# Plachtaa/FAcodec

Hardware: AMD Instinct MI355X
Metric: 24kHz audio sec encoded+decoded per wall-sec (higher is better)
Workload: dtype f32; 1 GPU; configs[1]: batch=32/GPU x 2 s @ 24 kHz, forward encoder->FVQ(6 codebooks)->decoder, FAcodec configs/config.yml model (137.7 M params), weights formula-generated, weight-norm re-materialised every step; clips_per_gpu=32, samples_per_clip=48000, parallelism=dp1 (independent clips, no collective)

## Files before the change

facodec_amd/_lib.py:

```python
import ctypes as C
import os

_HERE = os.path.dirname(os.path.abspath(__file__))
LIB_PATH = os.environ.get("FAC_LIB_PATH", os.path.join(_HERE, "libfacodec_hip.so"))

PAD_ZERO, PAD_REFLECT = 0, 1
ACT_NONE, ACT_TANH, ACT_MISH, ACT_LOG_MEL = 0, 1, 2, 3
ACT_GATE, ACT_WN_RES_SKIP = 4, 5

_p = C.c_void_p
_i = C.c_int
_i64 = C.c_int64
_f = C.c_float


class ConvDesc(C.Structure):
    _fields_ = [
        ("x", _p), ("w", _p), ("bias", _p), ("alpha_in", _p), ("alpha_out", _p), ("res", _p), ("y", _p), ("y2", _p), ("alpha_y2", _p), ("w_k1", _p), ("bias_k1", _p),
        ("x_bs", _i64), ("x_cs", _i64), ("y_bs", _i64), ("y_cs", _i64),
        ("B", C.c_int32), ("C_in", C.c_int32), ("T_in", C.c_int32), ("C_out", C.c_int32),
        ("C_out_pad", C.c_int32), ("T_out", C.c_int32),
        ("K", C.c_int32), ("stride", C.c_int32), ("dilation", C.c_int32), ("pad_left", C.c_int32),
        ("pad_mode", C.c_int32), ("n_phase", C.c_int32), ("y_tstride", C.c_int32), ("phase_shift", C.c_int32),
        ("act", C.c_int32),
        ("w_batched", C.c_int32), ("w_bs", _i64), ("ws", _p), ("ws_bytes", _i64), ("w_split", _p),
        ("K1", C.c_int32), ("dilation2", C.c_int32), ("row_phases", C.c_int32),
        ("x_p8", _p), ("x_p8_plane_bytes", _i64), ("y2_p8", _p), ("y2_p8_plane_bytes", _i64),
        ("pw_split", C.c_int32), ("split_rows", C.c_int32),
        ("gate_cond", _p), ("gate_cond_bs", _i64),
        ("keep_tile160", C.c_int32),
    ]


class VqDesc(C.Structure):
    _fields_ = [
        ("residual", _p), ("z_in", _p), ("zq_acc", _p), ("zq_out", _p), ("w_in", _p), ("b_in", _p),
        ("codebook", _p), ("w_out", _p), ("w_out_scale", _p), ("b_out", _p), ("mask", _p), ("codes", _p), ("z_e", _p),
        ("loss_part", _p), ("codes_bs", _i64),
        ("B", C.c_int32), ("D", C.c_int32), ("T", C.c_int32), ("Kc", C.c_int32),
    ]



VQ_DECODE_MAX_Q = 16


class VqDecodeDesc(C.Structure):
    _fields_ = [
        ("codes", _p * 3), ("codes_bs", _i64 * 3), ("codes_qs", _i64 * 3), ("n_q", C.c_int32 * 3),
        ("codebook", _p * VQ_DECODE_MAX_Q), ("w_out", _p * VQ_DECODE_MAX_Q), ("w_out_scale", _p * VQ_DECODE_MAX_Q),
        ("b_out", _p * VQ_DECODE_MAX_Q), ("style", _p), ("outs", _p), ("z", _p * 3),
        ("B", C.c_int32), ("D", C.c_int32), ("T", C.c_int32), ("Kc", C.c_int32),
    ]
# ... 120 lines not shown
    "fac_snake_bwd": (_i, [_p, _p, _p, _p, _p, _p, _i, _i, _i, _p]),
    "fac_pack_lstm_whh_t": (_i, [_p, _p, _i, _p]),
    "fac_lstm_layer_bwd": (_i, [_p, _p, _p, _p, _p, _p, _i, _i, _i, _p]),
    "fac_to_p8": (_i, [_p, _p, _p, _i, _i, _i, _p]),
    "fac_lstm_persist_ok": (_i, [_i, _i]),
    "fac_lstm_persist_stream_ok": (_i, [_p]),
    "fac_pack_lstm_whh16": (_i, [_p, _p, _i, _i, _p]),
    "fac_lstm_layer_fwd_persist": (_i, [_p, _p, _p, _p, _p, _p, _i, _i, _i, _i, _p]),
    "fac_lstm_layer_bwd_persist": (_i, [_p, _p, _p, _p, _p, _p, _i, _i, _i, _i, _p]),
    "fac_lstm_persist_split_ok": (_i, [_i, _i]),
    "fac_lstm_persist_timeouts": (_i, []),
    "fac_lstm_persist_arm": (_i, [_p]),
    "fac_lstm_abort_flag": (_i, [_p, _p]),
    "fac_mask_flags_if": (_i, [_p, _i, _p, _p]),
    "fac_pack_lstm_whh_split": (_i, [_p, _p, _i, _p]),
    "fac_lstm_layer_fwd_persist_split": (_i, [_p, _p, _p, _p, _i, _i, _i, _i, _p]),
    "fac_snake_bwd_fused": (_i, [_p, _p, _p, _p, _p, _p, _p, _p, _i, _i, _i, _p]),
    "fac_bias_grad": (_i, [_p, _p, _p, _i, _i, _i, _p]),
    "fac_snake_bwd_fused_rs": (_i, [_p, _p, _p, _i64, _p, _p, _p, _p, _p, _i, _i, _i, _p]),
    "fac_pad_fold_edges": (_i, [_p, _i, _i, _i, _i, _i, _p]),
    "fac_pack_convtr_w": (_i, [_p, _p, _p, _i, _i, _i, _i, _p]),
    "fac_conv1d_fwd": (_i, [C.POINTER(ConvDesc), _p]),
    "fac_conv1d_variant": (_i, [C.POINTER(ConvDesc), C.c_char_p, _i]),
    "fac_snake_fwd": (_i, [_p, _p, _p, _i, _i, _i, _p]),
    "fac_lstm_to_time_major": (_i, [_p, _p, _i, _i, _i, _p]),
    "fac_lstm_from_time_major": (_i, [_p, _p, _p, _p, _i, _i, _i, _p]),
    "fac_pack_lstm_whh": (_i, [_p, _p, _i, _p]),
    "fac_lstm_layer_fwd": (_i, [_p, _p, _p, _p, _i, _i, _i, _p]),
    "fac_lstm_layer_fwd_from": (_i, [_p, _p, _p, _p, _i, _i, _i, _i64, _p]),
    "fac_lstm_layer_fwd_train": (_i, [_p, _p, _p, _p, _p, _p, _i, _i, _i, _i64, _p]),
    "fac_lstm_gate_bwd": (_i, [_p, _p, _p, _p, _p, _p, _p, _i, _i, _i64, _i, _p]),
    "fac_tanh_bwd": (_i, [_p, _p, _p, _i64, _p]),
    "fac_pair_bwd": (_i, [_p, _p, _p, _i64, _i, C.c_float, C.c_float, _i, _p]),
    "fac_spec_power_bwd": (_i, [_p, _p, _p, _i, _i, _i, _i, _p]),
    "fac_stft_frames_bwd": (_i, [_p, _p, _i, _i, _i, _i, _i, _i, _i, _p]),
    "fac_vq_latent_bwd": (_i, [_p, _p, _p, _i64, _p, _p, _p, _p, _i, _i, _p]),
    "fac_vq_codebook_grad": (_i, [_p, _p, _p, _i64, _p, _p, _i, _i, _i, _i, _p]),
    "fac_layernorm_c_affine_bwd": (_i, [_p, _p, _p, _p, _p, _p, _i, _i, _i, _p]),
    "fac_rows_fma": (_i, [_p, _p, _p, _p, _i, _i64, _f, _p]),
    "fac_grad_norm_clip": (_i, [_p, _i64, _f, _p, _p, _p]),
    "fac_adamw_step": (_i, [_p, _p, _p, _p, _i64, _f, _f, _f, _f, _f, _i64, _p, _p]),
    "fac_logdiff_rms_bwd": (_i, [_p, _p, _p, _i, _i, _i, _f, _f, _i, _p]),
    "fac_gather_copy": (_i, [_p, _p, _p, _i, _p]),
    "fac_adamw_step_masked": (_i, [_p, _p, _p, _p, _i64, _p, _i, _p, _p, _p, _f, _f, _f, _f, _f, _p, _p]),
    "fac_gate_bwd": (_i, [_p, _p, _p, _i, _i, _i, _p]),
    "fac_mish_fwd": (_i, [_p, _p, _i64, _p]),
# ... 119 lines not shown
```

facodec_amd/build.py:

```python
import os
import subprocess
import sys
from concurrent.futures import ThreadPoolExecutor

HERE = os.path.dirname(os.path.abspath(__file__))
CSRC = os.path.join(HERE, "csrc")
TAG = os.environ.get("FAC_BUILD_TAG", "")
LIB = os.path.join(HERE, "libfacodec_hip%s.so" % ("_" + TAG if TAG else ""))
OBJDIR = "build" + ("_" + TAG if TAG else "")
SOURCES = ["conv1d_api.hip", "conv1d_tile_128x128.hip", "conv1d_tile_96x128.hip", "conv1d_tile_64x128.hip",
           "conv1d_tile_32x256.hip", "conv1d_tile_128x32.hip", "conv1d_tile_128x256.hip", "conv1d_fused_ru.hip", "conv1d_narrow.hip", "conv1d_pw.hip", "conv1d_pw_split.hip", "conv1d_skinny.hip", "conv1d_bsplit.hip", "conv1d_bsplit96.hip", "conv1d_gemm_split.hip", "conv1d_bsplit2.hip", "conv1d_bwd.hip", "conv1d_wgrad_split.hip", "conv1d_wgrad_k1.hip", "train_misc.hip", "optim.hip", "train_quant.hip", "train_pred.hip", "train_disc.hip", "train_redecoder.hip", "pack.hip", "prep_batch.hip", "lstm.hip", "lstm_persist.hip", "vq.hip", "vq_decode.hip", "bitpack.hip", "misc.hip", "attention_stream.hip", "attention_tiled.hip","ragged.hip", "resample.hip", "loudness.hip", "metrics.hip", "stream_pool.hip", "plc.hip", "jdc.hip", "rccl_arena.hip"]
FLAGS = ["--offload-arch=gfx950", "-O3", "-std=c++17", "-fPIC", "-ffp-contract=off",
         "-Wno-unused-result"] + os.environ.get("FAC_EXTRA_FLAGS", "").split()


def _hipcc():
    for cand in (os.environ.get("HIPCC"), "/opt/rocm/bin/hipcc", "hipcc"):
        if cand and (os.path.isabs(cand) and os.path.exists(cand) or not os.path.isabs(cand)):
            return cand
    return "hipcc"


def _stale(target, deps):
    if not os.path.exists(target):
        return True
    tt = os.path.getmtime(target)
    return any(os.path.getmtime(d) > tt for d in deps)


def build_lib(force=False, verbose=True):
    hipcc = _hipcc()
    headers = sorted(os.path.join(CSRC, f) for f in os.listdir(CSRC) if f.endswith(".h")) + [os.path.join(HERE, "..", "include", "facodec_hip.h")]
    objs, jobs = [], []
    os.makedirs(os.path.join(CSRC, OBJDIR), exist_ok=True)
# ... 23 lines not shown
```

facodec_amd/csrc/conv1d_api.hip:

```cpp
#include "conv1d_mfma.h"
#include <stdlib.h>

namespace fac {

enum ConvKernel : int {
  CK_128x32 = 0,
  CK_32x256 = 1,
  CK_64x128 = 2,
  CK_96x128 = 3,
  CK_128x128 = 4,
  CK_128x256 = 5,
  CK_96x256 = 6,
  CK_FUSED_RU = 7,
  CK_128x160 = 8,
  CK_NARROW = 9,
  CK_SKINNY = 10,
  CK_BSPLIT = 11,
  CK_CIN1 = 12,
  CK_THIN = 13,
  CK_PW = 14,
  CK_GSPLIT = 15,
  CK_BSPLIT2 = 16,
  CK_PWS = 17,
  CK_PWT = 18,
// ... 73 lines not shown
  {
    long long last = (long long)(d->T_out - 1) * d->stride + (long long)conv_max_tap_offset(a) - d->pad_left;
    int pad_right = last >= d->T_in ? (int)(last - d->T_in + 1) : 0;
    int max_pad = d->pad_left > pad_right ? d->pad_left : pad_right;
    a.T_ext = d->T_in > max_pad ? d->T_in : max_pad + 1;
  }
  if (d->x_p8 || d->y2_p8) {
    const bool gs = d->w_split && (d->K <= 2 || (d->stride > 1 && d->K <= 2 * d->stride)) && conv_gsplit_ok(a) &&
                    !conv_skinny_ok(a, d->ws, d->ws_bytes) && d->C_in % 8 == 0 && d->x_p8_plane_bytes < (1ll << 32);
    const bool ok = !d->y2_p8 && (gs || (d->w_split && !conv_two_level(a) && (d->split_rows == 96 ? conv_bsplit96_p8_ok(a) : conv_bsplit_p8_ok(a)) &&
                                       !conv_cin1_ok(a)));
    FAC_REQUIRE(ok, "conv1d: P8 operands given but the launch does not run on a kernel that takes them (K=%d stride=%d C_in=%d columns=%lld)",
                d->K, d->stride, d->C_in, (long long)d->B * d->T_out);
  }
  if (d->act == FAC_ACT_GATE || d->act == FAC_ACT_WN_RES_SKIP) {
    FAC_REQUIRE(d->w && !d->w_k1 && !d->x_p8 && !conv_two_level(a) && conv_skinny_ok(a, d->ws, d->ws_bytes),
                "conv1d: FAC_ACT_GATE / FAC_ACT_WN_RES_SKIP exist only for few-column launches (B * T_out <= 640) with a workspace");
    k = CK_SKINNY;
    return FAC_OK;
  }
  if (d->w_k1) { k = CK_FUSED_RU; return FAC_OK; }
  a.gflat = 0;
  a.grt = 0;
  if (d->w_split && (a.KV == 9 || a.KV == 3) && d->C_out <= 32 && conv_bsplit2_ok(a)) {
    a.w = reinterpret_cast<const float*>(d->w_split);
    k = CK_BSPLIT2;
    return FAC_OK;
  }
  FAC_REQUIRE(!conv_two_level(a) || d->w, "conv1d: two-level taps outside the split kernel's shapes need fp32 weights");
  const bool pw_on = pw_enabled();
  if (pw_on && d->pw_split && d->w && conv_pwt_ok(a)) { k = CK_PWT; return FAC_OK; }
  if (d->w_split && (d->K <= 2 || (d->stride > 1 && d->K <= 2 * d->stride)) && conv_gsplit_ok(a) &&
      !conv_skinny_ok(a, d->ws, d->ws_bytes)) {
    a.w = reinterpret_cast<const float*>(d->w_split);
    k = CK_GSPLIT;
    return FAC_OK;
  }
  if (a.rp > 1) {
    FAC_REQUIRE(d->w != nullptr && d->w != (const float*)d->w_split, "conv1d: row_phases launch outside the split kernel's shapes needs fp32 weights");
    k = CK_128x256;
    return FAC_OK;
  }
  const bool two_level = conv_two_level(a);
  FAC_REQUIRE(d->split_rows == 0 || d->split_rows == 64 || d->split_rows == 96, "conv1d: split_rows must be 0, 64 or 96");
  if (d->split_rows == 96) {
    FAC_REQUIRE(d->w_split && !two_level && conv_bsplit96_ok(a) && !conv_cin1_ok(a),
                "conv1d: split_rows = 96 needs a stride-1 k = 7 launch with C_out %% 96 == 0, C_in %% 8 == 0 and more than 640 columns "
                "(K=%d stride=%d C_in=%d C_out=%d columns=%lld)", d->K, d->stride, d->C_in, d->C_out, (long long)d->B * d->T_out);
    a.w = reinterpret_cast<const float*>(d->w_split);
    k = CK_BSPLIT96;
    return FAC_OK;
  }
  if (d->w_split && !two_level && conv_bsplit_ok(a) && !conv_cin1_ok(a)) {
    a.w = reinterpret_cast<const float*>(d->w_split);
    k = CK_BSPLIT;
    return FAC_OK;
  }
  FAC_REQUIRE(d->w != nullptr && (const void*)d->w != d->w_split,
// ... 13 lines not shown

extern "C" int fac_conv1d_fwd(const fac_conv_desc* d, fac_stream_t stream) {
  using namespace fac;
  ConvArgs a;
  ConvKernel k;
  if (const int rc = conv_plan(d, a, k)) return rc;
  hipStream_t s = (hipStream_t)stream;
  switch (k) {
    case CK_128x32: return conv_dispatch_128x32(a, s);
    case CK_32x256: return conv_dispatch_32x256(a, s);
    case CK_64x128: return conv_dispatch_64x128(a, s);
    case CK_96x128: return conv_dispatch_96x128(a, s);
    case CK_128x128: return conv_dispatch_128x128(a, s);
    case CK_128x256: return conv_dispatch_128x256(a, s);
    case CK_96x256: return conv_dispatch_96x256(a, s);
    case CK_FUSED_RU: return conv_dispatch_fused_ru(a, s);
    case CK_128x160: return conv_dispatch_128x160(a, s);
    case CK_NARROW: return conv_dispatch_narrow(a, s);
    case CK_SKINNY: return conv_dispatch_skinny(a, d->ws, d->ws_bytes, s);
    case CK_BSPLIT: return conv_dispatch_bsplit(a, s);
    case CK_CIN1: return conv_dispatch_cin1(a, s);
    case CK_THIN: return conv_dispatch_thin(a, d->ws, s);
    case CK_PW: return conv_dispatch_pw(a, s);
    case CK_GSPLIT: return conv_dispatch_gsplit(a, s);
    case CK_BSPLIT2: return conv_dispatch_bsplit2(a, s);
    case CK_PWS: return conv_dispatch_pws(a, s);
    case CK_PWT: return conv_dispatch_pwt(a, s);
    case CK_BSPLIT96: return conv_dispatch_bsplit96(a, s);
  }
  return FAC_ERR_ARG;
}

extern "C" int fac_conv1d_variant(const fac_conv_desc* d, char* name, int name_len) {
  using namespace fac;
  ConvArgs a;
  ConvKernel k;
  if (const int rc = conv_plan(d, a, k)) return rc;
  if (!name || name_len <= 0) return k;
  switch (k) {
    case CK_128x32: snprintf(name, name_len, "conv1d_mfma_kernel<1,1,4,1,K> 128x32"); break;
    case CK_32x256: snprintf(name, name_len, "conv1d_mfma_kernel<1,2,1,4,K> 32x256"); break;
    case CK_64x128: snprintf(name, name_len, "conv1d_mfma_kernel<2,1,1,4,K> 64x128"); break;
    case CK_96x128: snprintf(name, name_len, "conv1d_mfma_kernel<3,1,1,4,K> 96x128"); break;
    case CK_128x128: snprintf(name, name_len, "conv1d_mfma_kernel<2,2,2,2,K> 128x128"); break;
    case CK_128x256:
      snprintf(name, name_len, a.rp > 1 ? "conv1d_mfma_kernel<2,2,2,4,2> 128x256 (convtr, all phases per tile)" : "conv1d_mfma_kernel<2,2,2,4,K> 128x256");
      break;
    case CK_96x256: snprintf(name, name_len, "conv1d_mfma_kernel<3,1,1,8,K> 96x256"); break;
    case CK_FUSED_RU: snprintf(name, name_len, "conv1d_mfma_kernel<C/32,1,1,4,7,fused RU> Cx128"); break;
    case CK_128x160: snprintf(name, name_len, "conv1d_mfma_kernel<1,5,4,1,K> 128x160"); break;
    case CK_NARROW:
      snprintf(name, name_len, conv_two_level(a) ? "conv1d_narrow_kernel (VALU, C_out<=2, two-level taps)" : "conv1d_narrow_kernel (VALU, C_out<=2)");
      break;
    case CK_SKINNY:
      snprintf(name, name_len, conv_skinny_single_launch(a) ? "conv1d_gemv_kernel (single launch, <=4 columns)"
                                                            : "conv1d_skinny_kernel (split reduction, <=640 columns)");
      break;
    case CK_BSPLIT: snprintf(name, name_len, "conv1d_bsplit_kernel<%d> 64x256 (bf16x3 split, fp32-grade)", a.K); break;
    case CK_CIN1: snprintf(name, name_len, "conv1d_cin1_kernel (VALU, C_in=1, store stream)"); break;
    case CK_THIN: snprintf(name, name_len, "conv1d_thin_kernel (VALU, C_out<=8, split channels)"); break;
    case CK_PW: snprintf(name, name_len, "conv1d_pw_kernel (k=1 streaming, W in LDS)"); break;
    case CK_GSPLIT:
      snprintf(name, name_len, "conv1d_gemm_split_kernel<%d> 128x128 (bf16x3 split GEMM, fp32-grade)", a.stride > 1 ? 2 : a.K);
      break;
    case CK_BSPLIT2: snprintf(name, name_len, "conv1d_bsplit2_kernel<%d,%d> 32x512 (bf16x3 split, fp32-grade)", a.KV, a.stride); break;
    case CK_PWS: snprintf(name, name_len, "conv1d_pws_kernel (k=1 streaming, W planes in LDS, bf16x3 split, fp32-grade)"); break;
    case CK_PWT: snprintf(name, name_len, "conv1d_pwt_kernel<%d taps> (streaming, W planes in LDS, bf16x3 split, fp32-grade)", a.K); break;
    case CK_BSPLIT96: snprintf(name, name_len, "conv1d_bsplit_kernel<%d> 96x256 (bf16x3 split, fp32-grade)", a.K); break;
  }
  return k;
}
```

facodec_amd/csrc/conv1d_mfma.h:

```cpp
#pragma once
#include "common.h"

namespace fac {

typedef __attribute__((address_space(3))) void lds_void_t;
typedef __attribute__((address_space(1))) const void glb_void_t;

constexpr int CONV_XMAX = 6;

struct ConvArgs {
  const float* x;
  const float* w;
  const float* bias;
  const float* alpha_in;
  const float* alpha_out;
  const float* res;
  float* y;
  float* y2;
  const float* alpha2;
  const float* w1;
  const float* bias1;
  long long x_bs, x_cs, y_bs, y_cs, w_bs;
  int B, C_in, T_in, T_ext, C_out, C_out_pad, T_out;
  int K, stride, dil, pad_left, pad_mode;
  int n_phase, y_tstride, act, w_batched;
  int phase_shift;
  int K1, dil2;
  int K2v, KV, CV;
  int cic;
  int XW;
  int XB;
  int XQ, XR;
  int n_t_tiles;
  int n_tiles, persist;
  int x_off;
  int gflat;
  int grt;
  const unsigned char* x_p8;
  long long x_p8_ps;
  unsigned char* y2_p8;
  long long y2_p8_ps;
  int rp;
  const float* gate_cond;
  long long gate_cond_bs;
};

__host__ __device__ inline int conv_max_tap_offset(const ConvArgs& a) {
  const int K1 = (a.K1 > 0 && a.K1 < a.K) ? a.K1 : a.K;
  return (a.K / K1 - 1) * a.dil2 + (K1 - 1) * a.dil;
}
__host__ __device__ inline bool conv_two_level(const ConvArgs& a) { return a.K1 > 0 && a.K1 < a.K; }
inline void conv_set_virtual(ConvArgs& a) {
  a.KV = conv_two_level(a) ? a.K1 : a.K;
  a.K2v = a.K / a.KV;
  a.CV = a.C_in * a.K2v;
}

template <int KT>
struct ConvUnroll {
  static constexpr int UC = (KT == 1) ? 4 : ((KT == 2 || KT == 3) ? 2 : 1);
  static constexpr int CIC = KT == 1 ? 24 : (KT == 2 || KT == 3) ? 16 : (KT >= 4 && KT <= 7) ? 8 : (KT > 7 ? 4 : 0);
};

template <int KT, int T_TILE>
constexpr int conv_cic() {
  return ((KT == 2 || KT == 3) && T_TILE >= 256) ? 8 : ConvUnroll<KT>::CIC;
}
// ... 526 lines not shown
  return check_launch("conv1d_mfma");
}

int conv_dispatch_128x128(ConvArgs& a, hipStream_t s);
int conv_dispatch_96x128(ConvArgs& a, hipStream_t s);
int conv_dispatch_64x128(ConvArgs& a, hipStream_t s);
int conv_dispatch_32x256(ConvArgs& a, hipStream_t s);
int conv_dispatch_128x32(ConvArgs& a, hipStream_t s);
int conv_dispatch_128x256(ConvArgs& a, hipStream_t s);
int conv_dispatch_96x256(ConvArgs& a, hipStream_t s);
int conv_dispatch_fused_ru(ConvArgs& a, hipStream_t s);
int conv_dispatch_128x160(ConvArgs& a, hipStream_t s);
int conv_dispatch_narrow(ConvArgs& a, hipStream_t s);
bool conv_cin1_ok(const ConvArgs& a);
bool conv_pw_ok(const ConvArgs& a);
int conv_dispatch_pw(ConvArgs& a, hipStream_t s);
bool conv_thin_ok(const ConvArgs& a, const void* ws, long long ws_bytes);
int conv_dispatch_thin(ConvArgs& a, void* ws, hipStream_t s);
int conv_dispatch_cin1(ConvArgs& a, hipStream_t s);
bool conv_bsplit2_ok(const ConvArgs& a);
int conv_dispatch_bsplit2(ConvArgs& a, hipStream_t s);
bool conv_gsplit_ok(const ConvArgs& a);
int conv_dispatch_gsplit(ConvArgs& a, hipStream_t s);
bool conv_bsplit_ok(const ConvArgs& a);
bool conv_bsplit_p8_ok(const ConvArgs& a);
int conv_dispatch_bsplit(ConvArgs& a, hipStream_t s);
bool conv_bsplit96_ok(const ConvArgs& a);
bool conv_bsplit96_p8_ok(const ConvArgs& a);
int conv_dispatch_bsplit96(ConvArgs& a, hipStream_t s);
bool conv_pws_ok(const ConvArgs& a);
int conv_dispatch_pws(ConvArgs& a, hipStream_t s);
bool conv_pwt_ok(const ConvArgs& a);
int conv_dispatch_pwt(ConvArgs& a, hipStream_t s);
bool conv_skinny_ok(const ConvArgs& a, const void* ws, long long ws_bytes);
bool conv_skinny_single_launch(const ConvArgs& a);
int conv_dispatch_skinny(ConvArgs& a, void* ws, long long ws_bytes, hipStream_t s);

}
```

facodec_amd/csrc/misc.hip:

```cpp
#include "common.h"
#include <string.h>

namespace fac {

static thread_local char g_err[512] = "";

void set_error(const char* fmt, ...) {
  va_list ap;
  va_start(ap, fmt);
  vsnprintf(g_err, sizeof(g_err), fmt, ap);
  va_end(ap);
}

constexpr int EW_THREADS = 256;
inline int ew_grid(long long n, int per_thread = 1) {
  long long g = (n + (long long)EW_THREADS * per_thread - 1) / ((long long)EW_THREADS * per_thread);
  if (g > 8192) g = 8192;
  if (g < 1) g = 1;
  return (int)g;
}

__global__ void snake_kernel(const float* __restrict__ x, const float* __restrict__ alpha,
                             float* __restrict__ y, int C, int T, long long n) {
  for (long long i = (long long)blockIdx.x * blockDim.x + threadIdx.x; i < n;
// ... 547 lines not shown
    const float* pb = b + bb * M * T + t;
    float* pd = db + bb * M * T + t;
    float q = 0.f;
    for (int m = 0; m < M; ++m) {
      const float d = logf(fabsf(pa[(long long)m * T]) + eps) - logf(fabsf(pb[(long long)m * T]) + eps);
      q = fmaf(d, d, q);
    }
    const float r = sqrtf(q / (float)M);
    const float k = r > 0.f ? scale / ((float)M * r) : 0.f;
    for (int m = 0; m < M; ++m) {
      const float bv = pb[(long long)m * T];
      const float d = logf(fabsf(pa[(long long)m * T]) + eps) - logf(fabsf(bv) + eps);
      const float sg = bv > 0.f ? 1.f : (bv < 0.f ? -1.f : 0.f);
      const float g = -k * d * sg / (fabsf(bv) + eps);
      pd[(long long)m * T] = accumulate ? pd[(long long)m * T] + g : g;
    }
  }
}

}

using namespace fac;

extern "C" int fac_version(void) { return 5; }
extern "C" const char* fac_last_error(void) { return fac::g_err; }

#define EW_LAUNCH(kern, n, ...)                                                         \
  hipLaunchKernelGGL(kern, dim3(ew_grid(n)), dim3(EW_THREADS), 0, (hipStream_t)stream, __VA_ARGS__)

extern "C" int fac_snake_fwd(const float* x, const float* alpha, float* y, int B, int C, int T,
                             fac_stream_t stream) {
  FAC_REQUIRE(x && alpha && y && B > 0 && C > 0 && T > 0, "snake_fwd: bad arguments");
  const long long n = (long long)B * C * T;
  if (T >= 1024 && (long long)B * C <= 65535) {
    hipLaunchKernelGGL(snake_rows_kernel, dim3((T + 1023) / 1024, B * C), dim3(256), 0, (hipStream_t)stream, x, alpha, y, C, T);
  } else {
    EW_LAUNCH(snake_kernel, n, x, alpha, y, C, T, n);
  }
  return check_launch("snake_fwd");
}

extern "C" int fac_gate_tanh_sigmoid(const float* a, const float* g, int64_t g_bs, float* out, int B,
                                     int C, int T, fac_stream_t stream) {
  FAC_REQUIRE(a && out && B > 0 && C > 0 && T > 0, "gate_tanh_sigmoid: bad arguments");
  const long long n = (long long)B * C * T;
  EW_LAUNCH(gate_kernel, n, a, g, out, C, T, (long long)g_bs, n);
  return check_launch("gate_tanh_sigmoid");
// ... 245 lines not shown
```

facodec_amd/ops.py:

```python
import ctypes as C
import math
import os
from collections import namedtuple

import torch

from . import _lib
from .wprep import prepared
from .convplan import *
from ._lib import ConvDesc, VqDesc, VqDecodeDesc, ResampleDesc, PAD_REFLECT, PAD_ZERO, ACT_NONE, ACT_TANH, ACT_MISH, ACT_LOG_MEL, ACT_GATE, ACT_WN_RES_SKIP


def pad32(n):
    return (n + 31) & ~31


def cin_pad(c):
    return ((c + 47) // 48) * 48


_RAW_STREAM = getattr(torch._C, "_cuda_getCurrentRawStream", None)
_GET_DEVICE = getattr(torch._C, "_cuda_getDevice", None)


# ... 426 lines not shown

def conv_y_channels(c_out, act):
    return c_out // 2 if act in (ACT_GATE, ACT_WN_RES_SKIP) else c_out


def conv_desc(B, c_in, t_in, c_out, k, stride=1, dilation=1, pad_left=None, pad_mode=PAD_REFLECT, t_out=None, act=ACT_NONE, causal=True,
              k1=0, dilation2=0, c_out_pad=None, split_rows=0):
    if pad_left is None:
        t_o, padding_total, _ = conv_out_len(t_in, k, stride, dilation)
        pad_left = padding_total if causal else padding_total - padding_total // 2
        if t_out is None:
            t_out = t_o
    if t_out is None:
        raise ValueError("t_out required with explicit pad_left")
    d = ConvDesc()
    d.x_bs, d.x_cs = c_in * t_in, t_in
    d.y_bs, d.y_cs = conv_y_channels(c_out, act) * t_out, t_out
    d.B, d.C_in, d.T_in, d.C_out, d.C_out_pad, d.T_out = B, c_in, t_in, c_out, (pad32(c_out) if c_out_pad is None else c_out_pad), t_out
    d.K, d.stride, d.dilation, d.pad_left, d.pad_mode = k, stride, dilation, pad_left, pad_mode
    d.n_phase, d.y_tstride, d.act, d.w_batched, d.w_bs = 1, 1, act, 0, 0
    d.K1, d.dilation2, d.split_rows = k1, dilation2, split_rows
    d.pw_split = 1 if (BF16_SPLIT and PW_SPLIT and (k == 1 or (PW_TAPS and k == 4 and stride == 2))) else 0
    d.keep_tile160 = 0 if K1_COLUMN_TILES else 1
    return d


def conv1d(x, w_packed, c_out, k, bias=None, stride=1, dilation=1, pad_left=None, pad_mode=PAD_REFLECT,
           t_out=None, alpha_in=None, alpha_out=None, res=None, act=ACT_NONE, out=None, causal=True,
           alpha_y2=None, want_y=True, w_k1=None, bias_k1=None, w_split=None, k1=0, dilation2=0, skip_acc=None, gate_cond=None):
    x_p8 = x if isinstance(x, P8) else None
    if x_p8 is not None:
        B, c_in, t_in = x_p8.shape
    else:
        if not (x.is_cuda and x.dtype == torch.float32 and x.dim() == 3 and x.stride(2) == 1):
            x = _dev(x, "x")
        B, c_in, t_in = x.shape
    dev_ = x_p8.planes.device if x_p8 is not None else x.device
    d = conv_desc(B, c_in, t_in, c_out, k, stride, dilation, pad_left, pad_mode, t_out, act, causal, k1, dilation2,
                  w_packed.shape[-1] if w_packed is not None else None,
                  getattr(w_split, "split_rows", 0))
    t_out, c_y = d.T_out, conv_y_channels(c_out, act)
    if out is None and want_y:
        out = torch.empty(B, c_y, t_out, device=dev_, dtype=torch.float32)
    y2 = torch.empty(B, c_out, t_out, device=dev_, dtype=torch.float32) if alpha_y2 is not None else None
    if act == ACT_WN_RES_SKIP:
        assert skip_acc is not None and skip_acc.is_contiguous() and skip_acc.shape == out.shape and alpha_y2 is None
# ... 22 lines not shown
        if not (gate_cond.is_cuda and gate_cond.dtype == torch.float32 and gate_cond.dim() == 2 and gate_cond.shape == (B, c_out)
                and (gate_cond.stride(1) == 1 or c_out == 1)):
            raise ValueError(f"gate_cond must be a float32 GPU tensor (B={B}, c_out={c_out}) with contiguous rows, "
                             f"got {tuple(gate_cond.shape)} {gate_cond.dtype} {gate_cond.device}")
        d.gate_cond, d.gate_cond_bs = gate_cond.data_ptr(), gate_cond.stride(0)
    _launch_conv(d, "fac_conv1d_fwd")
    return (out, y2) if alpha_y2 is not None else out


STREAM_FOLD = True
SKINNY_MAX_COLS = 640


def convtr_desc(B, c_in, t_in, c_out, stride, c_out_pad, causal=True, has_history=False, rows=False, split=False):
    t_cols = t_in - 1 if has_history else t_in
    t_total = t_cols * stride
    d = ConvDesc()
    d.x_bs, d.x_cs = c_in * t_in, t_in
    d.y_bs, d.y_cs = c_out * t_total, t_total
    d.B, d.C_in, d.T_in, d.C_out, d.C_out_pad, d.T_out = B, c_in, t_in, c_out, c_out_pad, t_cols
    d.K, d.stride, d.dilation, d.pad_left, d.pad_mode = 2, 1, 1, (0 if has_history else 1), PAD_ZERO
    d.n_phase, d.y_tstride, d.act, d.w_batched, d.w_bs = stride, stride, ACT_NONE, 0, 0
    d.phase_shift = 0 if causal else stride - stride // 2
    if rows or split:
        if not causal or has_history:
            raise _lib.FacodecHipError("the all-phases ConvTranspose1d launch is causal and offline only")
        d.n_phase, d.y_tstride, d.phase_shift, d.row_phases = 1, 1, 0, stride
        d.pw_split = 1 if (BF16_SPLIT and PW_SPLIT and PW_TAPS and not split and stride == 2) else 0
    return d


def conv_transpose1d(x, w_packed, c_out, stride, bias=None, alpha_in=None, out=None, alpha_y2=None, causal=True,
                     has_history=False):
    x_p8 = x if isinstance(x, P8) else None
    if x_p8 is not None:
        assert not has_history
        B, c_in, t_in = x_p8.shape
    else:
        if not (has_history and x.is_cuda and x.dtype == torch.float32 and x.stride(2) == 1):
            x = _dev(x, "x")
        B, c_in, t_in = x.shape
    dev_ = x_p8.planes.device if x_p8 is not None else x.device
    if has_history:
        assert causal
    split_rows = isinstance(w_packed, tuple)
    d = convtr_desc(B, c_in, t_in, c_out, stride, w_packed[1] if split_rows else w_packed.shape[-1], causal, has_history,
# ... 3 lines not shown
    d.bias = bias.data_ptr() if bias is not None else None
    if x_p8 is not None:
        d.x, d.x_p8, d.x_p8_plane_bytes = None, x_p8.planes.data_ptr(), x_p8.plane_bytes
    else:
        d.x = x.data_ptr()
        d.x_bs, d.x_cs = x.stride(0), x.stride(1)
    if split_rows:
        d.w, d.w_split = None, w_packed[0].data_ptr()
    else:
        d.w = w_packed.data_ptr()
    d.alpha_in = alpha_in.data_ptr() if alpha_in is not None else None
    d.alpha_out, d.res, d.y = None, None, out.data_ptr()
    y2 = torch.empty_like(out) if alpha_y2 is not None else None
    d.y2 = y2.data_ptr() if y2 is not None else None
    d.alpha_y2 = alpha_y2.data_ptr() if alpha_y2 is not None else None
    _launch_conv(d, "fac_conv1d_fwd(convtr)")
    return (out, y2) if alpha_y2 is not None else out


FLAT_TRAIN = True
PW_SPLIT = os.environ.get("FAC_PW_SPLIT", "1") != "0"
PW_TAPS = True
K1_COLUMN_TILES = True


def pack_conv_for(layout, v, g, stride=1, k1=0, scale=None):
    if layout in (W_FP32, W_FP32_PW_TAPS):
        return pack_conv_weight(v, g, scale=scale), None
    if layout == W_GEMM_STRIDED:
        return None, pack_gemm_weight_split(v, g, in_stride=stride, scale=scale)
    if layout == W_SPLIT2:
        return None, pack_conv_weight_split2(v, g, k1, scale=scale)
    return None, pack_conv_weight_split(v, g, scale=scale, rows=64)


def pack_convtr_for(layout, v, g, stride):
    if layout in (TR_ROWS_SPLIT, TR_FLAT):
        return pack_convtr_weight_rows_split(v, g, stride)
    return pack_convtr_weight(v, g, stride) if layout == TR_POLYPHASE else pack_convtr_weight_rows(v, g, stride)


def convtr_weight_for(v, g, stride, t_in, causal=True, batch=1, alpha_in=None):
    return pack_convtr_for(plan_convtr(v.shape[0], v.shape[1], stride, batch, t_in, causal=causal, alpha_in=alpha_in is not None).layout,
                           v, g, stride)


# ... 1515 lines not shown
```

include/facodec_hip.h:

```cpp
#ifndef FACODEC_HIP_H
#define FACODEC_HIP_H

#include <stdint.h>

#ifdef __cplusplus
extern "C" {
#endif

typedef void* fac_stream_t;

#define FAC_OK 0
#define FAC_ERR_ARG (-1)
#define FAC_ERR_LAUNCH (-2)

#define FAC_PAD_ZERO 0
#define FAC_PAD_REFLECT 1

#define FAC_ACT_NONE 0
#define FAC_ACT_TANH 1
#define FAC_ACT_MISH 2
#define FAC_ACT_LOG_MEL 3
#define FAC_ACT_GATE 4
#define FAC_ACT_WN_RES_SKIP 5

// ... 36 lines not shown
  int32_t B, C_in, T_in, C_out, C_out_pad;
  int32_t T_out;
  int32_t K, stride, dilation, pad_left, pad_mode;
  int32_t n_phase;
  int32_t y_tstride;
  int32_t phase_shift;
  int32_t act;
  int32_t w_batched;
  int64_t w_bs;
  void* ws;
  int64_t ws_bytes;
  const void* w_split;
  int32_t K1, dilation2;
  int32_t row_phases;
  const void* x_p8;
  int64_t x_p8_plane_bytes;
  void* y2_p8;
  int64_t y2_p8_plane_bytes;
  int32_t pw_split;
  int32_t split_rows;
  const float* gate_cond;
  int64_t gate_cond_bs;
  int32_t keep_tile160;
} fac_conv_desc;

int fac_conv1d_fwd(const fac_conv_desc* d, fac_stream_t stream);
int fac_to_p8(const float* x, const float* alpha, void* out, int B, int C, int T, fac_stream_t stream);
int64_t fac_conv_w_split_bytes(int C_out, int C_in, int K);
int64_t fac_conv_w_split_rows_bytes(int C_out, int C_in, int K, int rows);
int fac_pack_conv_w_split_rows(const float* v, const float* scale, void* out, int C_out, int C_in, int K, int rows, fac_stream_t stream);
int fac_pack_conv_w_split(const float* v, const float* scale, void* out, int C_out, int C_in, int K,
                          fac_stream_t stream);
int64_t fac_conv_w_split2_bytes(int C_out, int C_in, int K, int K1);
int fac_pack_conv_w_split2(const float* v, const float* scale, void* out, int C_out, int C_in, int K, int K1, fac_stream_t stream);
int64_t fac_gemm_w_split_bytes(int R, int C_in, int K, int in_stride);
int fac_pack_gemm_w_split(const float* v, int64_t row_stride, int64_t ci_stride, int64_t k_stride, const float* row_scale, void* out,
                          int R, int C_in, int K, int in_stride, fac_stream_t stream);
int fac_conv1d_variant(const fac_conv_desc* d, char* name, int name_len);

int fac_snake_fwd(const float* x, const float* alpha, float* y, int B, int C, int T,
                  fac_stream_t stream);


int fac_lstm_to_time_major(const float* x, float* xT, int B, int H, int T, fac_stream_t stream);
int fac_lstm_from_time_major(const float* yT, const float* skip, const float* alpha, float* out, int B, int H, int T,
                             fac_stream_t stream);
int fac_pack_lstm_whh(const float* w_hh, float* packed, int H, fac_stream_t stream);
int fac_lstm_layer_fwd(const float* pre, const float* whh_packed, float* yT, float* c, int T,
                       int H, int BP, fac_stream_t stream);
// ... 394 lines not shown
```

Baseline: 1270 audio-s/s.

## Add P8-fragment bf16x3 split GEMM conv kernel with 64-row tiles and adaptive column width

Adds a new split-GEMM conv kernel that reads pre-split P8 activation fragments straight from global memory into registers, while streaming weights into LDS through a three-stage DMA ring. It uses 64-row tiles and picks between 128 and 256 columns with a wave-quantisation cost model, so two workgroups can fit per CU. The kernel is only used for large LSTM projections and ConvTranspose clip shapes when P8 input is available. This aims to improve occupancy and avoid separate activation-splitting work, but it adds another code path whose tile choice and register pressure could hurt some shapes.

New measurement: 1284 audio-s/s, median of 6. 1.01x the previous value.

```diff
diff --git a/facodec_amd/_lib.py b/facodec_amd/_lib.py
--- a/facodec_amd/_lib.py
+++ b/facodec_amd/_lib.py
@@ -28,7 +28,7 @@
         ("x_p8", _p), ("x_p8_plane_bytes", _i64), ("y2_p8", _p), ("y2_p8_plane_bytes", _i64),
         ("pw_split", C.c_int32), ("split_rows", C.c_int32),
         ("gate_cond", _p), ("gate_cond_bs", _i64),
-        ("keep_tile160", C.c_int32),
+        ("keep_tile160", C.c_int32), ("gsplit_p8_cols", C.c_int32),
     ]
 
 
@@ -195,6 +195,7 @@
     "fac_pack_convtr_w": (_i, [_p, _p, _p, _i, _i, _i, _i, _p]),
     "fac_conv1d_fwd": (_i, [C.POINTER(ConvDesc), _p]),
     "fac_conv1d_variant": (_i, [C.POINTER(ConvDesc), C.c_char_p, _i]),
+    "fac_gsplit_p8_tile_cols": (_i, [_i64, _i64, _i64, _i]),
     "fac_snake_fwd": (_i, [_p, _p, _p, _i, _i, _i, _p]),
     "fac_lstm_to_time_major": (_i, [_p, _p, _i, _i, _i, _p]),
     "fac_lstm_from_time_major": (_i, [_p, _p, _p, _p, _i, _i, _i, _p]),
diff --git a/facodec_amd/build.py b/facodec_amd/build.py
--- a/facodec_amd/build.py
+++ b/facodec_amd/build.py
@@ -9,7 +9,7 @@
 LIB = os.path.join(HERE, "libfacodec_hip%s.so" % ("_" + TAG if TAG else ""))
 OBJDIR = "build" + ("_" + TAG if TAG else "")
 SOURCES = ["conv1d_api.hip", "conv1d_tile_128x128.hip", "conv1d_tile_96x128.hip", "conv1d_tile_64x128.hip",
-           "conv1d_tile_32x256.hip", "conv1d_tile_128x32.hip", "conv1d_tile_128x256.hip", "conv1d_fused_ru.hip", "conv1d_narrow.hip", "conv1d_pw.hip", "conv1d_pw_split.hip", "conv1d_skinny.hip", "conv1d_bsplit.hip", "conv1d_bsplit96.hip", "conv1d_gemm_split.hip", "conv1d_bsplit2.hip", "conv1d_bwd.hip", "conv1d_wgrad_split.hip", "conv1d_wgrad_k1.hip", "train_misc.hip", "optim.hip", "train_quant.hip", "train_pred.hip", "train_disc.hip", "train_redecoder.hip", "pack.hip", "prep_batch.hip", "lstm.hip", "lstm_persist.hip", "vq.hip", "vq_decode.hip", "bitpack.hip", "misc.hip", "attention_stream.hip", "attention_tiled.hip","ragged.hip", "resample.hip", "loudness.hip", "metrics.hip", "stream_pool.hip", "plc.hip", "jdc.hip", "rccl_arena.hip"]
+           "conv1d_tile_32x256.hip", "conv1d_tile_128x32.hip", "conv1d_tile_128x256.hip", "conv1d_fused_ru.hip", "conv1d_narrow.hip", "conv1d_pw.hip", "conv1d_pw_split.hip", "conv1d_skinny.hip", "conv1d_bsplit.hip", "conv1d_bsplit96.hip", "conv1d_gemm_split.hip", "conv1d_gemm_split_p8.hip", "conv1d_bsplit2.hip", "conv1d_bwd.hip", "conv1d_wgrad_split.hip", "conv1d_wgrad_k1.hip", "train_misc.hip", "optim.hip", "train_quant.hip", "train_pred.hip", "train_disc.hip", "train_redecoder.hip", "pack.hip", "prep_batch.hip", "lstm.hip", "lstm_persist.hip", "vq.hip", "vq_decode.hip", "bitpack.hip", "misc.hip", "attention_stream.hip", "attention_tiled.hip","ragged.hip", "resample.hip", "loudness.hip", "metrics.hip", "stream_pool.hip", "plc.hip", "jdc.hip", "rccl_arena.hip"]
 FLAGS = ["--offload-arch=gfx950", "-O3", "-std=c++17", "-fPIC", "-ffp-contract=off",
          "-Wno-unused-result"] + os.environ.get("FAC_EXTRA_FLAGS", "").split()
 
diff --git a/facodec_amd/csrc/conv1d_api.hip b/facodec_amd/csrc/conv1d_api.hip
--- a/facodec_amd/csrc/conv1d_api.hip
+++ b/facodec_amd/csrc/conv1d_api.hip
@@ -119,6 +119,8 @@
   if (d->w_k1) { k = CK_FUSED_RU; return FAC_OK; }
   a.gflat = 0;
   a.grt = 0;
+  a.gs_ncb = 0;
+  a.gs_cols_req = 0;
   if (d->w_split && (a.KV == 9 || a.KV == 3) && d->C_out <= 32 && conv_bsplit2_ok(a)) {
     a.w = reinterpret_cast<const float*>(d->w_split);
     k = CK_BSPLIT2;
@@ -131,6 +133,12 @@
       !conv_skinny_ok(a, d->ws, d->ws_bytes)) {
     a.w = reinterpret_cast<const float*>(d->w_split);
     k = CK_GSPLIT;
+    if (d->x_p8) {
+      FAC_REQUIRE(d->gsplit_p8_cols == 0 || d->gsplit_p8_cols == -1 || d->gsplit_p8_cols == 128 || d->gsplit_p8_cols == 256,
+                  "conv1d: gsplit_p8_cols must be 0, -1, 128 or 256 (got %d)", d->gsplit_p8_cols);
+      a.gs_cols_req = d->gsplit_p8_cols;
+      a.gs_ncb = conv_gsplit_p8_ncb(a);
+    }
     return FAC_OK;
   }
   if (a.rp > 1) {
@@ -190,7 +198,7 @@
     case CK_CIN1: return conv_dispatch_cin1(a, s);
     case CK_THIN: return conv_dispatch_thin(a, d->ws, s);
     case CK_PW: return conv_dispatch_pw(a, s);
-    case CK_GSPLIT: return conv_dispatch_gsplit(a, s);
+    case CK_GSPLIT: return a.gs_ncb ? conv_dispatch_gsplit_p8(a, s) : conv_dispatch_gsplit(a, s);
     case CK_BSPLIT2: return conv_dispatch_bsplit2(a, s);
     case CK_PWS: return conv_dispatch_pws(a, s);
     case CK_PWT: return conv_dispatch_pwt(a, s);
@@ -229,7 +237,8 @@
     case CK_THIN: snprintf(name, name_len, "conv1d_thin_kernel (VALU, C_out<=8, split channels)"); break;
     case CK_PW: snprintf(name, name_len, "conv1d_pw_kernel (k=1 streaming, W in LDS)"); break;
     case CK_GSPLIT:
-      snprintf(name, name_len, "conv1d_gemm_split_kernel<%d> 128x128 (bf16x3 split GEMM, fp32-grade)", a.stride > 1 ? 2 : a.K);
+      if (a.gs_ncb) snprintf(name, name_len, "conv1d_gemm_split_kernel<%d> 64x%d (bf16x3 split GEMM, fp32-grade, P8 fragments)", a.stride > 1 ? 2 : a.K, 64 * a.gs_ncb);
+      else snprintf(name, name_len, "conv1d_gemm_split_kernel<%d> 128x128 (bf16x3 split GEMM, fp32-grade)", a.stride > 1 ? 2 : a.K);
       break;
     case CK_BSPLIT2: snprintf(name, name_len, "conv1d_bsplit2_kernel<%d,%d> 32x512 (bf16x3 split, fp32-grade)", a.KV, a.stride); break;
     case CK_PWS: snprintf(name, name_len, "conv1d_pws_kernel (k=1 streaming, W planes in LDS, bf16x3 split, fp32-grade)"); break;
diff --git a/facodec_amd/csrc/conv1d_gemm_split_p8.hip b/facodec_amd/csrc/conv1d_gemm_split_p8.hip
--- /dev/null
+++ b/facodec_amd/csrc/conv1d_gemm_split_p8.hip
@@ -0,0 +1,383 @@
+#include "conv1d_mfma.h"
+
+namespace fac {
+
+constexpr int GP_ROWS = 64;
+constexpr int GP_PACK_ROWS = 128;
+constexpr int GP_RB = 64;
+constexpr int GP_BLK = GP_ROWS * GP_RB;
+constexpr int GP_NST = 3;
+constexpr int GP_D = 2;
+
+__host__ __device__ constexpr int gp_stage_bytes(int K) { return 3 * K * GP_BLK; }
+__host__ __device__ constexpr size_t gp_lds_bytes(int K, int NCB) {
+  const size_t st = (size_t)GP_NST * gp_stage_bytes(K), epi = (size_t)GP_ROWS * (64 * NCB + 4) * sizeof(float);
+  return st > epi ? st : epi;
+}
+static_assert(gp_lds_bytes(2, 4) <= 80 * 1024 && gp_lds_bytes(1, 4) <= 80 * 1024, "two workgroups must fit the 160 KB of a CU");
+
+__device__ __forceinline__ void gp_dma16(const unsigned char* src, unsigned lds) {
+  unsigned keep;
+  asm volatile("s_mov_b32 %0, m0\n\ts_mov_b32 m0, %2\n\ts_nop 0\n\tglobal_load_lds_dwordx4 %1, off\n\ts_mov_b32 m0, %0"
+               : "=&s"(keep) : "v"(src), "s"(lds) : "memory");
+}
+
+typedef const __attribute__((address_space(1))) bf16x8 glb_bf16x8;
+
+template <int RPT, int COLS>
+__device__ __forceinline__ void gp_epilogue(const ConvArgs& a, const float* tile, int tid, int rt64, int n0, int b, bool flat,
+                                            long long n_total) {
+  constexpr int EP = COLS + 4;
+  const int rp = RPT > 0 ? RPT : a.rp;
+  const int cpt = GP_PACK_ROWS / rp;
+  const int QPR = (COLS * rp) / 4;
+  const int h64 = (rt64 & 1) * GP_ROWS;
+  const int ch_base = (rt64 >> 1) * cpt;
+  const int cl_lo = h64 / rp;
+  int cl_hi = (h64 + GP_ROWS - 1) / rp;
+  cl_hi = cl_hi < cpt - 1 ? cl_hi : cpt - 1;
+  const int nq = (cl_hi - cl_lo + 1) * QPR;
+  const long long u_tot = n_total * rp;
+  const long long u0 = (long long)n0 * rp;
+  const bool al_ok = (a.y_cs & 3) == 0 && (a.y_bs & 3) == 0 && (!a.y || (reinterpret_cast<unsigned long long>(a.y) & 15) == 0) &&
+                     (!a.y2 || (reinterpret_cast<unsigned long long>(a.y2) & 15) == 0) &&
+                     (!a.res || (reinterpret_cast<unsigned long long>(a.res) & 15) == 0) && (!flat || (a.T_out & 3) == 0);
+  for (int q = tid; q < nq; q += 256) {
+    const int cq = q / QPR, uq = q - cq * QPR;
+    const int cl = cl_lo + cq;
+    const int co = ch_base + cl;
+    const long long u = u0 + 4 * uq;
+    if (co >= a.C_out || u >= u_tot) continue;
+    float v[4];
+    bool own[4] = {true, true, true, true};
+    if (RPT == 1) {
+      const float4 av = *reinterpret_cast<const float4*>(tile + (cl - h64) * EP + 4 * uq);
+      v[0] = av.x; v[1] = av.y; v[2] = av.z; v[3] = av.w;
+    } else {
+#pragma unroll
+      for (int i = 0; i < 4; ++i) {
+        const int ul = 4 * uq + i, tl = ul / rp, p = ul - tl * rp;
+        const int lr = cl * rp + p - h64;
+        own[i] = lr >= 0 && lr < GP_ROWS;
+        v[i] = own[i] ? tile[lr * EP + tl] : 0.f;
+      }
+    }
+    const bool own_all = own[0] && own[1] && own[2] && own[3];
+    long long o, lim = u_tot - u;
+    if (flat) {
+      const long long bb = u / a.T_out, tt = u - bb * a.T_out;
+      o = bb * a.y_bs + (long long)co * a.y_cs + tt;
+      const long long in_clip = a.T_out - tt;
+      lim = lim < in_clip ? lim : in_clip;
+    } else {
+      o = (long long)b * a.y_bs + (long long)co * a.y_cs + u;
+    }
+    const bool full = al_ok && lim >= 4 && own_all;
+    const float bs = a.bias ? a.bias[co] : 0.f;
+    const float al = a.alpha_out ? a.alpha_out[co] : 0.f;
+    const float inv = a.alpha_out ? snake_inv(al) : 0.f;
+    if (flat && lim < 4) {
+#pragma unroll
+      for (int i = 0; i < 4; ++i) {
+        const long long ui = u + i;
+        if (ui >= u_tot || !own[i]) continue;
+        const long long bb = ui / a.T_out, tt = ui - bb * a.T_out;
+        const long long oi = bb * a.y_bs + (long long)co * a.y_cs + tt;
+        float x = v[i] + bs;
+        if (a.alpha_out) x = snake_apply(x, al, inv);
+        if (a.act != FAC_ACT_NONE) x = apply_act_slow(x, a.act);
+        if (a.res) x += a.res[oi];
+        if (a.y) a.y[oi] = x;
+        if (a.y2) { const float a2 = a.alpha2[co]; a.y2[oi] = snake_apply(x, a2, snake_inv(a2)); }
+      }
+      continue;
+    }
+    float rv[4] = {0.f, 0.f, 0.f, 0.f};
+    if (a.res) {
+      if (full) {
+        const float4 r4 = *reinterpret_cast<const float4*>(a.res + o);
+        rv[0] = r4.x; rv[1] = r4.y; rv[2] = r4.z; rv[3] = r4.w;
+      } else {
+#pragma unroll
+        for (int i = 0; i < 4; ++i) rv[i] = (i < lim && own[i]) ? a.res[o + i] : 0.f;
+      }
+    }
+#pragma unroll
+    for (int i = 0; i < 4; ++i) {
+      float x = v[i] + bs;
+      if (a.alpha_out) x = snake_apply(x, al, inv);
+      if (a.act != FAC_ACT_NONE) x = apply_act_slow(x, a.act);
+      v[i] = x + rv[i];
+    }
+    float w[4] = {0.f, 0.f, 0.f, 0.f};
+    if (a.y2) {
+      const float a2 = a.alpha2[co], i2 = snake_inv(a2);
+#pragma unroll
+      for (int i = 0; i < 4; ++i) w[i] = snake_apply(v[i], a2, i2);
+    }
+    if (full) {
+      if (a.y) *reinterpret_cast<float4*>(a.y + o) = make_float4(v[0], v[1], v[2], v[3]);
+      if (a.y2) *reinterpret_cast<float4*>(a.y2 + o) = make_float4(w[0], w[1], w[2], w[3]);
+    } else {
+#pragma unroll
+      for (int i = 0; i < 4; ++i) {
+        if (i >= lim || !own[i]) continue;
+        if (a.y) a.y[o + i] = v[i];
+        if (a.y2) a.y2[o + i] = w[i];
+      }
+    }
+  }
+}
+
+template <int K, int NCB>
+__global__ __launch_bounds__(256, 2) void conv1d_gemm_split_p8_kernel(ConvArgs a) {
+  constexpr int COLS = 64 * NCB;
+  constexpr int NBW = NCB / 2;
+  constexpr int STAGE = gp_stage_bytes(K);
+  constexpr int PACK_CHUNK = 3 * K * GP_PACK_ROWS * GP_RB;
+  constexpr int NSTEP = 2 * K;
+  constexpr int RING = GP_D + 1;
+  constexpr int LB = 3 * NBW;
+  constexpr int NA = 3 * K;
+  static_assert(GP_D <= NSTEP && (GP_NST * NSTEP) % RING == 0, "static ring slots need NST * NSTEP to be a multiple of the ring");
+  extern __shared__ __attribute__((aligned(16))) unsigned char sm[];
+  const int tid = threadIdx.x;
+  const int lane = tid & 63;
+  const int wave = __builtin_amdgcn_readfirstlane(tid >> 6);
+  const bool flat = a.gflat != 0;
+
+  int n0, rt64, b;
+  {
+    const int id = xcd_contiguous_id<unsigned>(blockIdx.x, gridDim.x);
+    const int nt = a.n_t_tiles, nb = flat ? 1 : a.B;
+    if (a.grt > 0) {
+      rt64 = id % a.grt;
+      const int rest = id / a.grt;
+      n0 = (rest % nt) * COLS;
+      b = rest / nt;
+    } else {
+      n0 = (id % nt) * COLS;
+      const int rest = id / nt;
+      b = rest % nb;
+      rt64 = rest / nb;
+    }
+  }
+  const int S = (K == 2 && a.stride > 1) ? a.stride : 1;
+  const int n_chunks = ((a.C_in + 31) / 32) * S;
+  const long long n_total = flat ? (long long)a.B * a.T_out : (long long)a.T_out;
+
+  const int l31 = lane & 31, kq = lane >> 5;
+  const int C8 = a.C_in / 8;
+  const unsigned zero_off = (unsigned)(((long long)a.B * C8 * a.T_in) * 16);
+  const unsigned grp_bytes = (unsigned)a.T_in * 16u;
+  const unsigned clip_off = flat ? 0u : (unsigned)((((long long)b * C8) * a.T_in) * 16);
+
+  const unsigned lds0 = __builtin_amdgcn_readfirstlane((unsigned)(size_t)(lds_void_t*)sm);
+  const unsigned char* wsrc = reinterpret_cast<const unsigned char*>(a.w) + (long long)(rt64 >> 1) * n_chunks * PACK_CHUNK +
+                              (rt64 & 1) * GP_BLK + wave * 1024 + lane * 16;
+  auto issue_a = [&](int chunk, int buf) {
+    const unsigned char* src = wsrc + (long long)chunk * PACK_CHUNK;
+    const unsigned dst = lds0 + buf * STAGE + wave * 1024;
+#pragma unroll
+    for (int j = 0; j < NA; ++j) gp_dma16(src + j * (GP_PACK_ROWS * GP_RB), dst + j * GP_BLK);
+  };
+
+  unsigned coff[NBW][K];
+#pragma unroll
+  for (int n = 0; n < NBW; ++n)
+#pragma unroll
+    for (int k = 0; k < K; ++k) {
+      const int r = wave * (32 * NBW) + n * 32 + l31 + k;
+      unsigned off = zero_off;
+      if (flat) {
+        const long long nn = (long long)n0 + r;
+        if (nn < n_total) {
+          const long long bb = nn / a.T_out;
+          off = (unsigned)(((bb * C8) * a.T_in + (nn - bb * a.T_out)) * 16);
+        }
+      } else if (S == 1) {
+        const int tin = n0 - a.pad_left + r;
+        if (tin >= 0 && tin < a.T_in) off = clip_off + (unsigned)tin * 16u;
+      } else {
+        off = (unsigned)r;
+      }
+      coff[n][k] = off;
+    }
+  auto col_off = [&](int n, int k, int ph) -> unsigned {
+    if (S == 1) return coff[n][k];
+    const int tin = (n0 + (int)coff[n][k]) * S + ph - a.pad_left;
+    int idx;
+    if (a.pad_mode == FAC_PAD_REFLECT) idx = reflect_index(tin, a.T_in, a.T_ext);
+    else idx = (tin >= 0 && tin < a.T_in) ? tin : -1;
+    return idx >= 0 ? clip_off + (unsigned)idx * 16u : zero_off;
+  };
+  const unsigned char* pl[3];
+#pragma unroll
+  for (int p = 0; p < 3; ++p) pl[p] = a.x_p8 + (long long)p * a.x_p8_ps;
+  auto ld_b = [&](int chunk, int step, bf16x8 (&Bf)[NBW][3]) {
+    const int k = step >> 1, ks = step & 1;
+    const int c32 = chunk / S, ph = chunk - c32 * S;
+    int g8 = c32 * 4 + ks * 2 + kq;
+    g8 = g8 < C8 ? g8 : C8 - 1;
+#pragma unroll
+    for (int n = 0; n < NBW; ++n) {
+      const unsigned off = col_off(n, k, ph);
+      const unsigned goff = off == zero_off ? zero_off : off + (unsigned)g8 * grp_bytes;
+#pragma unroll
+      for (int p = 0; p < 3; ++p) Bf[n][p] = *(glb_bf16x8*)(pl[p] + goff);
+    }
+  };
+
+  const int swa = (l31 >> 2) & 3;
+  int apo[2];
+#pragma unroll
+  for (int ks = 0; ks < 2; ++ks) apo[ks] = l31 * GP_RB + (((ks * 2 + kq) ^ swa) * 16);
+  auto ld_a = [&](const unsigned char* st, int step, bf16x8 (&A)[2][3]) {
+    const int k = step >> 1, ks = step & 1;
+#pragma unroll
+    for (int p = 0; p < 3; ++p)
+#pragma unroll
+      for (int m = 0; m < 2; ++m) A[m][p] = *reinterpret_cast<const bf16x8*>(st + (p * K + k) * GP_BLK + m * 32 * GP_RB + apo[ks]);
+  };
+
+  f32x16 acc[2][NBW];
+#pragma unroll
+  for (int m = 0; m < 2; ++m)
+#pragma unroll
+    for (int n = 0; n < NBW; ++n)
+#pragma unroll
+      for (int r = 0; r < 16; ++r) acc[m][n][r] = 0.f;
+
+  bf16x8 A[2][2][3], Bf[RING][NBW][3];
+  issue_a(0, 0);
+  if (n_chunks > 1) issue_a(1, 1);
+#pragma unroll
+  for (int s = 0; s < GP_D; ++s) ld_b(s / NSTEP, s % NSTEP, Bf[s]);
+
+  for (int base = 0; base < n_chunks; base += GP_NST) {
+#pragma unroll
+    for (int i = 0; i < GP_NST; ++i) {
+      const int c = base + i;
+      if (c >= n_chunks) break;
+      {
+        if (c + 1 < n_chunks) asm volatile("s_waitcnt vmcnt(%0)" : : "n"(NA + GP_D * LB) : "memory");
+        else asm volatile("s_waitcnt vmcnt(%0)" : : "n"(GP_D * LB) : "memory");
+        wg_barrier();
+        if (c + 2 < n_chunks) issue_a(c + 2, (i + 2) % GP_NST);
+        const unsigned char* st = sm + i * STAGE;
+        ld_a(st, 0, A[0]);
+#pragma unroll
+        for (int step = 0; step < NSTEP; ++step) {
+          const int gs = i * NSTEP + step;
+          {
+            const int s2 = step + GP_D;
+            const int c2 = c + s2 / NSTEP;
+            ld_b(c2 < n_chunks ? c2 : n_chunks - 1, s2 % NSTEP, Bf[(gs + GP_D) % RING]);
+          }
+          if (step + 1 < NSTEP) ld_a(st, step + 1, A[(step + 1) & 1]);
+          __builtin_amdgcn_sched_barrier(0);
+          constexpr int TA[6] = {1, 2, 0, 1, 0, 0}, TB[6] = {1, 0, 2, 0, 1, 0};
+#pragma unroll
+          for (int q = 0; q < 6; ++q)
+#pragma unroll
+            for (int m = 0; m < 2; ++m)
+#pragma unroll
+              for (int n = 0; n < NBW; ++n)
+                acc[m][n] = __builtin_amdgcn_mfma_f32_32x32x16_bf16(A[step & 1][m][TA[q]], Bf[gs % RING][n][TB[q]], acc[m][n], 0, 0, 0);
+          __builtin_amdgcn_sched_barrier(0);
+        }
+      }
+    }
+  }
+  wg_barrier();
+
+  {
+    float* tile = reinterpret_cast<float*>(sm);
+    constexpr int EP = COLS + 4;
+#pragma unroll
+    for (int m = 0; m < 2; ++m)
+#pragma unroll
+      for (int n = 0; n < NBW; ++n)
+#pragma unroll
+        for (int r = 0; r < 16; ++r)
+          tile[(m * 32 + (r & 3) + 8 * (r >> 2) + 4 * kq) * EP + wave * (32 * NBW) + n * 32 + l31] = acc[m][n][r];
+  }
+  __syncthreads();
+  const float* tile = reinterpret_cast<const float*>(sm);
+  switch (a.rp) {
+    case 1: gp_epilogue<1, COLS>(a, tile, tid, rt64, n0, b, flat, n_total); break;
+    case 2: gp_epilogue<2, COLS>(a, tile, tid, rt64, n0, b, flat, n_total); break;
+    case 5: gp_epilogue<5, COLS>(a, tile, tid, rt64, n0, b, flat, n_total); break;
+    case 6: gp_epilogue<6, COLS>(a, tile, tid, rt64, n0, b, flat, n_total); break;
+    default: gp_epilogue<0, COLS>(a, tile, tid, rt64, n0, b, flat, n_total); break;
+  }
+}
+
+
+int gp_choose_ncb(long long n_rt64, long long cols, long long nb, int slots) {
+  long long cost[2];
+  for (int i = 0; i < 2; ++i) {
+    const int w = i == 0 ? 256 : 128;
+    const long long n_wg = n_rt64 * ((cols + w - 1) / w) * nb;
+    cost[i] = ((n_wg + slots - 1) / slots) * w;
+  }
+  return cost[1] < cost[0] ? 2 : 4;
+}
+
+static int gp_slots() {
+  const int cus = device_cus();
+  return 2 * (cus > 0 ? cus : 256);
+}
+
+int conv_gsplit_p8_ncb(const ConvArgs& a) {
+  if (a.x_p8 == nullptr || a.gs_cols_req < 0 || a.C_in % 8 != 0) return 0;
+  if (a.gs_cols_req > 0) return a.gs_cols_req / 64;
+  const bool lstm_proj = a.K == 1 && a.stride == 1 && a.rp == 1 && a.C_in >= 1024 && a.C_out >= 4096;
+  const bool convtr_clips = a.K == 2 && a.stride == 1 && a.rp > 1 && a.B > 1 && a.C_in >= 384 && a.T_out >= 960;
+  if (!lstm_proj && !convtr_clips) return 0;
+  const bool flat = a.K == 1 && a.stride == 1;
+  const int rows = a.rp > 1 ? a.C_out_pad : a.C_out;
+  return gp_choose_ncb((rows + GP_ROWS - 1) / GP_ROWS, flat ? (long long)a.B * a.T_out : (long long)a.T_out, flat ? 1 : a.B, gp_slots());
+}
+
+template <int K, int NCB>
+static int gp_launch(ConvArgs& a, hipStream_t s) {
+  constexpr auto kern = conv1d_gemm_split_p8_kernel<K, NCB>;
+  allow_dynamic_lds<kern>(80 * 1024);
+  a.gflat = (K == 1) ? 1 : 0;
+  const long long n_total = a.gflat ? (long long)a.B * a.T_out : (long long)a.T_out;
+  a.n_t_tiles = (int)((n_total + 64 * NCB - 1) / (64 * NCB));
+  const int rows = a.rp > 1 ? a.C_out_pad : a.C_out;
+  const int n_rt = (rows + GP_ROWS - 1) / GP_ROWS;
+  const long long n_wg = (long long)a.n_t_tiles * n_rt * (a.gflat ? 1 : a.B);
+  {
+    const double x_bytes = 6.0 * a.B * a.C_in * (double)a.T_in;
+    const double w_bytes = 6.0 * rows * (double)a.C_in * K * (a.stride > 1 && K == 2 ? a.stride : 1);
+    const double n_ct = (double)a.n_t_tiles * (a.gflat ? 1 : a.B);
+    const double g = 64.0 / n_rt > 1.0 ? 64.0 / n_rt : 1.0;
+    const double slow = x_bytes * n_rt + w_bytes;
+    const double fast = x_bytes + (w_bytes <= 3.5 * 1048576.0 ? 8.0 * w_bytes : w_bytes * n_ct / g);
+    a.grt = (n_rt > 1 && fast < 0.8 * slow) ? n_rt : 0;
+  }
+  if (n_wg > 0x7fffffffll) {
+    set_error("conv1d(gemm split, P8 fragments): too many workgroups (%lld)", n_wg);
+    return FAC_ERR_ARG;
+  }
+  hipLaunchKernelGGL(kern, dim3((unsigned)n_wg), dim3(256), gp_lds_bytes(K, NCB), s, a);
+  return check_launch("conv1d_gemm_split_p8");
+}
+
+int conv_dispatch_gsplit_p8(ConvArgs& a, hipStream_t s) {
+  const bool k1 = a.K == 1 && a.stride == 1;
+  if (a.gs_ncb == 4) return k1 ? gp_launch<1, 4>(a, s) : gp_launch<2, 4>(a, s);
+  if (a.gs_ncb == 2) return k1 ? gp_launch<1, 2>(a, s) : gp_launch<2, 2>(a, s);
+  set_error("conv1d(gemm split, P8 fragments): no form with %d column blocks", a.gs_ncb);
+  return FAC_ERR_ARG;
+}
+
+}
+
+extern "C" int fac_gsplit_p8_tile_cols(int64_t rows, int64_t cols, int64_t ranges, int slots) {
+  if (rows <= 0 || cols <= 0 || ranges <= 0 || slots <= 0) return 0;
+  return 64 * fac::gp_choose_ncb((rows + fac::GP_ROWS - 1) / fac::GP_ROWS, cols, ranges, slots);
+}
diff --git a/facodec_amd/csrc/conv1d_mfma.h b/facodec_amd/csrc/conv1d_mfma.h
--- a/facodec_amd/csrc/conv1d_mfma.h
+++ b/facodec_amd/csrc/conv1d_mfma.h
@@ -43,6 +43,8 @@
   int rp;
   const float* gate_cond;
   long long gate_cond_bs;
+  int gs_ncb;
+  int gs_cols_req;
 };
 
 __host__ __device__ inline int conv_max_tap_offset(const ConvArgs& a) {
@@ -615,6 +617,8 @@
 int conv_dispatch_bsplit2(ConvArgs& a, hipStream_t s);
 bool conv_gsplit_ok(const ConvArgs& a);
 int conv_dispatch_gsplit(ConvArgs& a, hipStream_t s);
+int conv_gsplit_p8_ncb(const ConvArgs& a);
+int conv_dispatch_gsplit_p8(ConvArgs& a, hipStream_t s);
 bool conv_bsplit_ok(const ConvArgs& a);
 bool conv_bsplit_p8_ok(const ConvArgs& a);
 int conv_dispatch_bsplit(ConvArgs& a, hipStream_t s);
diff --git a/facodec_amd/csrc/misc.hip b/facodec_amd/csrc/misc.hip
--- a/facodec_amd/csrc/misc.hip
+++ b/facodec_amd/csrc/misc.hip
@@ -593,7 +593,7 @@
 
 using namespace fac;
 
-extern "C" int fac_version(void) { return 5; }
+extern "C" int fac_version(void) { return 6; }
 extern "C" const char* fac_last_error(void) { return fac::g_err; }
 
 #define EW_LAUNCH(kern, n, ...)                                                         \
diff --git a/facodec_amd/ops.py b/facodec_amd/ops.py
--- a/facodec_amd/ops.py
+++ b/facodec_amd/ops.py
@@ -472,6 +472,7 @@
     d.K1, d.dilation2, d.split_rows = k1, dilation2, split_rows
     d.pw_split = 1 if (BF16_SPLIT and PW_SPLIT and (k == 1 or (PW_TAPS and k == 4 and stride == 2))) else 0
     d.keep_tile160 = 0 if K1_COLUMN_TILES else 1
+    d.gsplit_p8_cols = GSPLIT_P8_COLS
     return d
 
 
@@ -540,6 +541,7 @@
     d.K, d.stride, d.dilation, d.pad_left, d.pad_mode = 2, 1, 1, (0 if has_history else 1), PAD_ZERO
     d.n_phase, d.y_tstride, d.act, d.w_batched, d.w_bs = stride, stride, ACT_NONE, 0, 0
     d.phase_shift = 0 if causal else stride - stride // 2
+    d.gsplit_p8_cols = GSPLIT_P8_COLS
     if rows or split:
         if not causal or has_history:
             raise _lib.FacodecHipError("the all-phases ConvTranspose1d launch is causal and offline only")
@@ -589,6 +591,7 @@
 PW_SPLIT = os.environ.get("FAC_PW_SPLIT", "1") != "0"
 PW_TAPS = True
 K1_COLUMN_TILES = True
+GSPLIT_P8_COLS = 0
 
 
 def pack_conv_for(layout, v, g, stride=1, k1=0, scale=None):
diff --git a/include/facodec_hip.h b/include/facodec_hip.h
--- a/include/facodec_hip.h
+++ b/include/facodec_hip.h
@@ -82,9 +82,11 @@
   const float* gate_cond;
   int64_t gate_cond_bs;
   int32_t keep_tile160;
+  int32_t gsplit_p8_cols;
 } fac_conv_desc;
 
 int fac_conv1d_fwd(const fac_conv_desc* d, fac_stream_t stream);
+int fac_gsplit_p8_tile_cols(int64_t rows, int64_t cols, int64_t ranges, int slots);
 int fac_to_p8(const float* x, const float* alpha, void* out, int B, int C, int T, fac_stream_t stream);
 int64_t fac_conv_w_split_bytes(int C_out, int C_in, int K);
 int64_t fac_conv_w_split_rows_bytes(int C_out, int C_in, int K, int rows);
```
